# tatsuya-ogawa/GaussianSplattingMlx

Measured on AMD Instinct MI355X. Metric: train views/sec (full step: fwd + L1/DSSIM loss + bwd + Adam + densify/prune at the reference cadence), Lego 800x800 300k Gaussians, higher is better.
Workload: dtype f32

## Files before the change

gaussiansplattingmlx_amd/csrc/blend_v2.hip:

```cpp
#include "gs_ctx.h"
#include "gs_bwd_prep.h"
#include "gs_cull.h"
#include "gs_wavesum.h"

namespace gs {

constexpr int BLK = 16;
constexpr uint32_t CKPT_POOL_MAX = 8;
static inline uint32_t ckpt_pool(uint32_t partSlots, uint32_t waves)
{
    const uint32_t perWave = partSlots / (waves / 8u + 1u);
    return perWave >= CKPT_POOL_MAX ? CKPT_POOL_MAX : (perWave < 1u ? 1u : perWave);
}

struct Rec {
    float mx, my, c00, c01, c10, c11, r, g, b, op, depth;
};

#ifndef GS_FWD_PREFETCH
#define GS_FWD_PREFETCH 1
#endif

typedef float f4 __attribute__((ext_vector_type(4)));
typedef float f2 __attribute__((ext_vector_type(2)));
// ... 587 lines not shown
        const int by = b / blocksX, bx = b - by * blocksX;
        const int tile = ((by * BLK) / tileH) * gridW + (bx * BLK) / tileW;
        const uint32_t start = __builtin_amdgcn_readfirstlane(tileRanges[2 * tile]);
        const uint32_t end = __builtin_amdgcn_readfirstlane(tileRanges[2 * tile + 1]);
        const uint32_t count = end > start ? end - start : 0u;
        const uint32_t sbase = __builtin_amdgcn_readfirstlane(segBase[b]);

        int X0, Y0, XL, YL;
        gs_block_pixels(vg, bx, by, W, H, X0, Y0, XL, YL);
        const int x = X0 + k * 8 + (lane & 7), y = Y0 + h * 8 + (lane >> 3);
        const bool in = x < XL && y < YL;
        const float px = (float)x, py = (float)y;
        const float qx0 = (float)(X0 + k * 8), qx1 = qx0 + 7.0f, qy0 = (float)(Y0 + h * 8), qy1 = qy0 + 7.0f;
        float T = in ? 1.0f : 0.0f;
        float cr = 0.f, cg = 0.f, cb = 0.f, dd = 0.f;
        uint32_t nc = 0;

        const uint32_t* __restrict__ idx = sortedIdx + start;
        auto save_state_vals = [&](uint32_t i, float sT, float sr, float sgr, float sb, float sd) {
            if (poolNext == poolEnd) {
                poolNext = qslotCap;
                for (uint32_t t = 0; t < 8u && poolNext == qslotCap; t++) {
                    const uint32_t yy = (part + t) & 7u;
                    if ((partsEmpty >> yy) & 1u) continue;
                    uint32_t base = 0;
                    if (lane == 0) base = atomicAdd(&counters[GS_CNT_QSLOTS + yy], ckptPool);
                    base = __builtin_amdgcn_readfirstlane(base);
                    if (base + ckptPool <= qslotPart) poolNext = gridDim.x * 4u * qslotOwn + yy * qslotPart + base;
                    else {
                        partsEmpty |= 1u << yy;
                        if (lane == 0) atomicSub(&counters[GS_CNT_QSLOTS + yy], ckptPool);
                    }
                }
                if (poolNext == qslotCap && partsEmpty == 0xFFu && lane == 0) atomicAdd(&counters[GS_CNT_QSLOTS + part], ckptPool);
                poolEnd = poolNext + ckptPool;
            }
            const uint32_t phys = poolNext++;
            const uint32_t vslot = sbase + i / SEG - 1;
            if (phys < qslotCap && vslot < segCap) {
                if (lane == 0) segSlot[(size_t)vslot * 4 + (h * 2 + k)] = phys;
                float* st = segState + (size_t)phys * (statePlanes * 64) + lane;
                if (sT >= 1e-4f) {
                    st[0] = sT; st[64] = sr; st[128] = sgr; st[192] = sb;
                    if (DEPTH && statePlanes == 5) st[256] = sd;
                }
            } else if (lane == 0) {
                counters[GS_CNT_OVERFLOW] = 1u;
                hostWords[4] = 2u;
            }
        };
        auto save_state = [&](uint32_t i) { save_state_vals(i, T, cr, cg, cb, dd); };
        struct Pre {
            float aclamp, r, g, b, depth;
            uint32_t ncv;
        };
        auto stage_compact = [&](f4* sl, const RecV& v, uint32_t c0) -> uint32_t {
            const float qmin = rect_min_q(v.a.z, v.a.w, v.b.x, v.b.y, qx0 - v.a.x, qx1 - v.a.x, qy0 - v.a.y, qy1 - v.a.y);
            const bool keep = (c0 + lane < count) && !(qmin > CULL_QMIN);
            const unsigned long long m = __ballot(keep);
            const uint32_t ps = (uint32_t)__popcll(m & ((1ull << lane) - 1ull));
            if (keep) {
                sl[ps * 3] = v.a; sl[ps * 3 + 1] = v.b;
                sl[ps * 3 + 2] = (f4){v.c.x, v.c.y, v.c.z, __uint_as_float(c0 + (uint32_t)lane + 1u)};
            }
            const uint32_t n = (uint32_t)__popcll(m), n4 = (n + 3u) & ~3u;
            if ((uint32_t)lane < n4 - n) {
                const f4 z = (f4){0.f, 0.f, 0.f, 0.f};
                sl[(n + lane) * 3] = z; sl[(n + lane) * 3 + 1] = z;
                sl[(n + lane) * 3 + 2] = (f4){0.f, 0.f, 0.f, __uint_as_float(min(c0 + 64u, count))};
            }
            return n4;
        };
        auto pre = [&](const f4* sl, uint32_t j, Pre& o) {
            const Rec s = unpack(sl[j * 3], sl[j * 3 + 1], sl[j * 3 + 2]);
            const float dx = px - s.mx, dy = py - s.my;
            const float dxdy = dx * dy, dx2 = dx * dx, dy2 = dy * dy;
            const float q = ((dx2 * s.c00 + dy2 * s.c11) + dxdy * s.c01) + dxdy * s.c10;
            o.aclamp = fminf(gauss_alpha_raw(q, s.op), 0.99f);
            o.r = s.r; o.g = s.g; o.b = s.b; o.depth = s.depth;
            o.ncv = __float_as_uint(sl[j * 3 + 2].w);
        };
        auto post = [&](const Pre& o) {
            const bool a = T >= 1e-4f;
            nc = a ? o.ncv : nc;
            const float alpha = a ? o.aclamp : 0.0f;
            const float wgt = T * alpha;
            cr = fmaf(wgt, o.r, cr); cg = fmaf(wgt, o.g, cg); cb = fmaf(wgt, o.b, cb); if (DEPTH) dd = fmaf(wgt, o.depth, dd);
            T = T * (1.0f - alpha);
        };
        auto any_live = [&]() { return __any(T >= 1e-4f); };
        auto trips_abs = [&](const f4* sl, uint32_t n, uint32_t c0, float* park) {
            park[lane] = cr; park[64 + lane] = cg; park[128 + lane] = cb; if (DEPTH) park[192 + lane] = dd;
            cr = 0.f; cg = 0.f; cb = 0.f; dd = 0.f;
            bool live = true;
            for (uint32_t j = 0; j < n && live; j += 4) {
                Pre p0, p1, p2, p3;
                pre(sl, j, p0); pre(sl, j + 1, p1); pre(sl, j + 2, p2); pre(sl, j + 3, p3);
                post(p0); post(p1); post(p2); post(p3);
                live = any_live();
            }
            if (live && T >= 1e-4f) nc = min(c0 + 64u, count);
            cr = park[lane] + cr; cg = park[64 + lane] + cg; cb = park[128 + lane] + cb; if (DEPTH) dd = park[192 + lane] + dd;
        };

        auto chunk_of = [&](uint32_t r) { return 256u * r + 64u * (((uint32_t)hw + r) & 3u); };
        RecV nx = load_chunk(rec12, idx, idxMask, chunk_of(0), count, lane);
        uint32_t gN = load_chunk_index(idx, idxMask, chunk_of(1), count, lane);
        for (uint32_t r = 0; 256u * r < count; r++) {
            if (!any_live()) break;
            const uint32_t s0 = 256u * r;
            const int w = (int)(((uint32_t)hw + r) & 3u);
            const uint32_t c0 = s0 + 64u * (uint32_t)w;
            const uint32_t nParts = min(4u, (count - s0 + 63u) / 64u);
            const bool mine = (uint32_t)w < nParts;
            f4* sl = sg;
            uint32_t n = 0;
            if (mine) n = stage_compact(sl, nx, c0);
            nx = gather_chunk(rec12, gN);
            gN = load_chunk_index(idx, idxMask, chunk_of(r + 2), count, lane);
            if (w == 0) {
                if (statePlanes != 0 && c0 != 0) save_state(c0);
                trips_abs(sl, n, c0, &xPre[hw][0][0]);
            } else if (mine) {
                T = in ? 1.0f : 0.0f; cr = 0.f; cg = 0.f; cb = 0.f; dd = 0.f;
                for (uint32_t j = 0; j < n; j += 4) {
                    Pre p0, p1, p2, p3;
                    pre(sl, j, p0); pre(sl, j + 1, p1); pre(sl, j + 2, p2); pre(sl, j + 3, p3);
#pragma unroll
                    for (int u = 0; u < 4; u++) {
                        const Pre& o = u == 0 ? p0 : u == 1 ? p1 : u == 2 ? p2 : p3;
                        const float wgt = T * o.aclamp;
                        cr = fmaf(wgt, o.r, cr); cg = fmaf(wgt, o.g, cg); cb = fmaf(wgt, o.b, cb); if (DEPTH) dd = fmaf(wgt, o.depth, dd);
                        T = T * (1.0f - o.aclamp);
                    }
                }
            }
            if (mine) { xEnd[w][0][lane] = T; xEnd[w][1][lane] = cr; xEnd[w][2][lane] = cg; xEnd[w][3][lane] = cb; xEnd[w][4][lane] = dd; }
            if (w == 0) xDead[0][5][lane] = __uint_as_float(nc);
            __syncthreads();
            float PT = xEnd[0][0][lane], Pr = xEnd[0][1][lane], Pg = xEnd[0][2][lane], Pb = xEnd[0][3][lane], Pd = xEnd[0][4][lane];
            uint32_t Pnc = __float_as_uint(xDead[0][5][lane]);
            float myPT = 0.0f;
            uint32_t qDone = 1;
            for (;;) {
                int crossedIn = 0;
#pragma unroll
                for (int q = 1; q < 4; q++) {
                    if ((uint32_t)q >= qDone && (uint32_t)q < nParts && !crossedIn) {
                        if (q == w) { myPT = PT; xPre[hw][0][lane] = Pr; xPre[hw][1][lane] = Pg; xPre[hw][2][lane] = Pb; if (DEPTH) xPre[hw][3][lane] = Pd; }
                        if (PT >= 1e-4f) {
                            const float Tend = PT * xEnd[q][0][lane];
                            if (Tend * foldScale >= 1e-4f) {
                                Pr = fmaf(PT, xEnd[q][1][lane], Pr); Pg = fmaf(PT, xEnd[q][2][lane], Pg); Pb = fmaf(PT, xEnd[q][3][lane], Pb);
                                if (DEPTH) Pd = fmaf(PT, xEnd[q][4][lane], Pd);
                                PT = Tend;
                                Pnc = min(s0 + 64u * (uint32_t)(q + 1), count);
                            } else crossedIn = q;
                        }
                        if (!crossedIn) qDone = (uint32_t)q + 1u;
                    }
                }
                if (!__syncthreads_or(crossedIn != 0)) break;
                if (w != 0 && mine && __any(crossedIn == w)) {
                    T = crossedIn == w ? PT : 0.0f; cr = Pr; cg = Pg; cb = Pb; dd = Pd; nc = 0;
                    trips_abs(sl, n, c0, &xDead[w][1][0]);
                    if (crossedIn == w) {
                        xDead[w][0][lane] = T; xDead[w][1][lane] = cr; xDead[w][2][lane] = cg; xDead[w][3][lane] = cb; xDead[w][4][lane] = dd;
                        xDead[w][5][lane] = __uint_as_float(nc);
                    }
                }
                __syncthreads();
                bool again = false;
                if (crossedIn) {
                    PT = xDead[crossedIn][0][lane]; Pr = xDead[crossedIn][1][lane]; Pg = xDead[crossedIn][2][lane];
                    Pb = xDead[crossedIn][3][lane]; Pd = xDead[crossedIn][4][lane]; Pnc = __float_as_uint(xDead[crossedIn][5][lane]);
                    qDone = (uint32_t)crossedIn + 1u;
                    again = PT >= 1e-4f && qDone < nParts;
                    if (!again) qDone = 4u;
                }
                if (!__syncthreads_or(again)) break;
            }
            if (statePlanes != 0 && w != 0 && mine && __any(myPT >= 1e-4f))
                save_state_vals(c0, myPT, xPre[hw][0][lane], xPre[hw][1][lane], xPre[hw][2][lane], DEPTH ? xPre[hw][3][lane] : 0.0f);
            T = PT; cr = Pr; cg = Pg; cb = Pb; dd = Pd; nc = Pnc;
        }
        if (hw == 0) {
            if (cutStore && any_live() && lane == 0 && cutStore[tile] != 0u) hostWords[0] = 1u;
            const int xe = X0 + k * 8 + (lane & 7), ye = Y0 + h * 8 + (lane >> 3);
            if (xe < XL && ye < YL) {
                const size_t pix = (size_t)ye * W + xe;
                float bg0, bg1, bg2;
                gs_bg_terms(bgc, T, bg0, bg1, bg2);
                outColor[3 * pix] = cr + bg0; outColor[3 * pix + 1] = cg + bg1; outColor[3 * pix + 2] = cb + bg2;
                if (DEPTH) outDepth[pix] = dd;
                outAlpha[pix] = 1.0f - T; lastContrib[pix] = nc; finalT[pix] = T;
            }
            uint32_t m = (xe < XL && ye < YL) ? nc : 0u;
#pragma unroll
            for (int d = 32; d >= 1; d >>= 1) m = max(m, (uint32_t)__shfl_xor((int)m, d, 64));
            if (lane == 0 && m) atomicMax(&blockWork[b], m);
        }
    }
}


struct RecB {
    float mx, my, A, B, Dq, r, g, b, op, depth;
};
__device__ __forceinline__ RecB unpack_b(const f4 a, const f4 b, const f4 c)
{
    RecB r;
    r.mx = a.x; r.my = a.y; r.A = a.z; r.B = a.w;
    r.Dq = b.x; r.r = b.z; r.g = b.w;
    r.b = c.x; r.op = c.y; r.depth = c.z;
    return r;
}
constexpr float EXP_INV_C1 = -1.3862943611198906f;

struct PairB {
    f2 dx, dxdy, dx2, e2;
    float dy, dy2;
};
__device__ __forceinline__ void pair_exponent_bwd(const RecB& s, f2 px, float py, PairB& o)
{
    o.dx = px - splat2(s.mx);
    o.dy = py - s.my;
    o.dxdy = o.dx * splat2(o.dy);
    o.dx2 = o.dx * o.dx;
    o.dy2 = o.dy * o.dy;
    o.e2 = fma2(o.dxdy, splat2(s.B), fma2(o.dx2, splat2(s.A), splat2(o.dy2 * s.Dq)));
}

struct PairState {
    f2 px, Ts, Q;
    f2 cCx, cCy, cCz, cD;
    float py;
    uint32_t nc0, nc1;
};

template <bool DEPTH, bool ABSGRAD, int NACC>
__device__ __forceinline__ void pair_bwd(const RecB& s, uint32_t i, const PairB& e, PairState& p, f2 (&acc)[NACC])
{
    static_assert(NACC == (ABSGRAD ? 12 : 10), "ten sums, twelve with the absolute ones");
    const f2 G = (f2){__builtin_amdgcn_exp2f(e.e2.x), __builtin_amdgcn_exp2f(e.e2.y)};
    const f2 raw = splat2(s.op) * G;
    const bool a0 = i < p.nc0, a1 = i < p.nc1;
    f2 alpha;
    alpha.x = a0 ? fminf(raw.x, 0.99f) : 0.0f;
    alpha.y = a1 ? fminf(raw.y, 0.99f) : 0.0f;
    const f2 contrib = p.Ts * alpha;
    const f2 S = fma2(p.cCx, splat2(s.r), fma2(p.cCy, splat2(s.g),
                      DEPTH ? fma2(p.cCz, splat2(s.b), p.cD * splat2(s.depth)) : p.cCz * splat2(s.b)));
    p.Q = fma2(-contrib, S, p.Q);
    const f2 oma = splat2(1.0f) - alpha;
    const f2 owed = p.Q * (f2){__builtin_amdgcn_rcpf(oma.x), __builtin_amdgcn_rcpf(oma.y)};
    const f2 dAlpha = fma2(p.Ts, S, -owed);
    f2 gate;
    gate.x = (a0 && !(raw.x > 0.99f)) ? dAlpha.x : 0.0f;
    gate.y = (a1 && !(raw.y > 0.99f)) ? dAlpha.y : 0.0f;
    const f2 hh = gate * raw;
    acc[0] = fma2(hh, e.dx, acc[0]);
    acc[1] = fma2(hh, splat2(e.dy), acc[1]);
    acc[2] = fma2(e.dx2, hh, acc[2]);
    acc[3] = fma2(e.dxdy, hh, acc[3]);
    acc[4] = fma2(splat2(e.dy2), hh, acc[4]);
    acc[5] = fma2(G, gate, acc[5]);
    acc[6] = fma2(contrib, p.cCx, acc[6]);
    acc[7] = fma2(contrib, p.cCy, acc[7]);
    acc[8] = fma2(contrib, p.cCz, acc[8]);
    if (DEPTH) acc[9] = fma2(contrib, p.cD, acc[9]);
    if constexpr (ABSGRAD) {
        const float hB = 0.5f * s.B;
        const float tx = hB * e.dy, ty = s.Dq * e.dy;
        const float u0 = fmaf(e.dx.x, s.A, tx), u1 = fmaf(e.dx.y, s.A, tx);
        const float v0 = fmaf(e.dx.x, hB, ty), v1 = fmaf(e.dx.y, hB, ty);
        acc[10].x = fmaf(fabsf(hh.x), fabsf(u0), acc[10].x);
        acc[10].y = fmaf(fabsf(hh.y), fabsf(u1), acc[10].y);
        acc[11].x = fmaf(fabsf(hh.x), fabsf(v0), acc[11].x);
        acc[11].y = fmaf(fabsf(hh.y), fabsf(v1), acc[11].y);
    }
    p.Ts = p.Ts * oma;
}

template <int SEG, bool DEPTH, bool ABSGRAD>
__global__ __launch_bounds__(64) void blend_bwd_v2_kernel(
    int W, int H, int tileW, int tileH, int gridW, int blocksX, GsBackground bgc, const float4* __restrict__ rec12,
    const uint32_t* __restrict__ sortedIdx, uint32_t idxMask, const uint32_t* __restrict__ tileRanges,
    const uint32_t* __restrict__ itemRow, const uint4* __restrict__ segSlot, uint32_t qslotCap, int statePlanes,
    const uint32_t* __restrict__ blockWork,
    const uint32_t* __restrict__ itemBlock, uint32_t* __restrict__ counters, uint32_t* __restrict__ bwdQueue, uint32_t nq,
    const float* __restrict__ cotColor,
    const float* __restrict__ cotDepth, const float* __restrict__ cotAlpha, const float* __restrict__ outColor,
    const float* __restrict__ outDepth, const float* __restrict__ outAlpha, const uint32_t* __restrict__ lastContrib,
    const float* __restrict__ finalT, const float* __restrict__ segState, float* __restrict__ gradAcc16, GsVirtGeom vg)
{
    __shared__ float part[SEG][16];
    __shared__ f4 sg[192];
    const int lane = threadIdx.x;
    const uint32_t nItems = __builtin_amdgcn_readfirstlane(counters[GS_CNT_ITEMS]);
    const uint32_t xcd = blockIdx.x % nq, slot = blockIdx.x / nq;
    const uint32_t perQ = (nItems + nq - 1u) / nq;
    const uint32_t staticPerQ = min(gridDim.x / nq, perQ);
    uint32_t dead = 0;
    for (bool first = true;; first = false) {
        uint32_t item = 0xFFFFFFFFu;
        if (first && slot < staticPerQ) item = xcd * perQ + slot;
        else {
            for (uint32_t t = 0; t < nq && item == 0xFFFFFFFFu; t++) {
                const uint32_t y = (xcd + t) % nq;
                if ((dead >> y) & 1u) continue;
                uint32_t k = 0;
                if (lane == 0) k = atomicAdd(&bwdQueue[y * 32u], 1u);
                k = __builtin_amdgcn_readfirstlane(k);
                const uint32_t idx = staticPerQ + k;
                if (idx < perQ && y * perQ + idx < nItems) item = y * perQ + idx;
                else dead |= 1u << y;
            }
        }
        if (item == 0xFFFFFFFFu || item >= nItems) {
            if (first) continue;
            break;
        }
        const uint32_t packed = __builtin_amdgcn_readfirstlane(itemBlock[item]);
        const uint32_t row = __builtin_amdgcn_readfirstlane(itemRow[item]);
        const int b = (int)(packed >> 10);
        const uint32_t seg = packed & 1023u;
        const int by = b / blocksX, bx = b - by * blocksX;
        const int tile = ((by * BLK) / tileH) * gridW + (bx * BLK) / tileW;
        const uint32_t start = __builtin_amdgcn_readfirstlane(tileRanges[2 * tile]);
        const uint32_t work = __builtin_amdgcn_readfirstlane(blockWork[b]);
        const uint32_t i0 = seg * SEG, i1 = min(i0 + SEG, work);
        uint32_t qslot[4] = {0, 0, 0, 0};
        if (seg != 0) {
            const uint4 q4 = segSlot[row];
            qslot[0] = __builtin_amdgcn_readfirstlane(q4.x); qslot[1] = __builtin_amdgcn_readfirstlane(q4.y);
            qslot[2] = __builtin_amdgcn_readfirstlane(q4.z); qslot[3] = __builtin_amdgcn_readfirstlane(q4.w);
        }

        int BX0, BY0, BXL, BYL;
        gs_block_pixels(vg, bx, by, W, H, BX0, BY0, BXL, BYL);
        PairState ps[2];
#pragma unroll
        for (int h = 0; h < 2; h++) {
            PairState& p = ps[h];
            const int y = BY0 + h * 8 + (lane >> 3);
            p.py = (float)y;
            p.Ts = p.Q = p.cCx = p.cCy = p.cCz = p.cD = splat2(0.f);
            uint32_t ncs[2] = {0, 0};
#pragma unroll
            for (int k = 0; k < 2; k++) {
                const int x = BX0 + k * 8 + (lane & 7);
                p.px[k] = (float)x;
                if (x < BXL && y < BYL) {
                    const size_t pix = (size_t)y * W + x;
                    const uint32_t n = lastContrib[pix];
                    if (n > i0) {
                        ncs[k] = n;
                        const float gx = cotColor[3 * pix], gy = cotColor[3 * pix + 1], gz = cotColor[3 * pix + 2];
                        const float gd = DEPTH ? cotDepth[pix] : 0.0f;
                        p.cCx[k] = gx; p.cCy[k] = gy; p.cCz[k] = gz; p.cD[k] = gd;
                        const float cA = cotAlpha ? cotAlpha[pix] : 0.0f;
                        const float Tn = finalT[pix];
                        float bg0, bg1, bg2;
                        gs_bg_terms(bgc, Tn, bg0, bg1, bg2);
                        const float cTn = -cA + gs_bg_cot(bgc, gx, gy, gz);
                        const float sc = (1.0f - outAlpha[pix]) / Tn;
                        float T0 = 1.0f, s0 = 0.0f, s1 = 0.0f, s2 = 0.0f, s3 = 0.0f;
                        const uint32_t phys = qslot[h * 2 + k];
                        if (seg != 0 && phys < qslotCap) {
                            const float* st = segState + (size_t)phys * (statePlanes * 64) + lane;
                            T0 = st[0]; s0 = st[64]; s1 = st[128]; s2 = st[192];
                            if (DEPTH) s3 = st[256];
                        }
                        const float d0 = (outColor[3 * pix] - bg0) - s0, d1 = (outColor[3 * pix + 1] - bg1) - s1, d2 = (outColor[3 * pix + 2] - bg2) - s2;
                        const float owedC = fmaf(gx, d0, fmaf(gy, d1, fmaf(gz, d2, DEPTH ? gd * (outDepth[pix] - s3) : 0.0f)));
                        p.Ts[k] = sc * T0;
                        p.Q[k] = sc * (owedC + Tn * cTn);
                    }
                }
            }
            p.nc0 = ncs[0]; p.nc1 = ncs[1];
        }

        uint32_t hm0 = max(ps[0].nc0, ps[0].nc1), hm1 = max(ps[1].nc0, ps[1].nc1);
#pragma unroll
        for (int d = 32; d >= 1; d >>= 1) {
            hm0 = max(hm0, (uint32_t)__shfl_xor((int)hm0, d, 64));
            hm1 = max(hm1, (uint32_t)__shfl_xor((int)hm1, d, 64));
        }
        const uint32_t* __restrict__ idx = sortedIdx + start;
        const uint32_t n = i1 - i0;
        for (uint32_t r = lane; r < n * 4; r += 64) reinterpret_cast<f4*>(&part[0][0])[r] = (f4){0.f, 0.f, 0.f, 0.f};
        const float bx0 = (float)BX0, bx1 = bx0 + 15.0f, by0 = (float)BY0;
        for (uint32_t c0 = i0; c0 < i1; c0 += 64) {
            uint32_t nEff;
            {
                const RecV v = load_chunk(rec12, idx, idxMask, c0, i1, lane);
                const float X0 = bx0 - v.a.x, X1 = bx1 - v.a.x, Yt = by0 - v.a.y;
                const uint32_t li = c0 + (uint32_t)lane;
                const bool far0 = li >= hm0 || rect_min_q(v.a.z, v.a.w, v.b.x, v.b.y, X0, X1, Yt, Yt + 7.0f) > CULL_QMIN;
                const bool far1 = li >= hm1 || rect_min_q(v.a.z, v.a.w, v.b.x, v.b.y, X0, X1, Yt + 8.0f, Yt + 15.0f) > CULL_QMIN;
                const bool keep = (c0 + lane < i1) && !(far0 && far1);
                const unsigned long long m = __ballot(keep);
                const uint32_t pos = (uint32_t)__popcll(m & ((1ull << lane) - 1ull));
                if (keep) {
                    const uint32_t tag = (c0 - i0 + (uint32_t)lane) | (far0 ? 256u : 0u) | (far1 ? 512u : 0u);
                    sg[pos * 3] = (f4){v.a.x, v.a.y, v.a.z * EXP_C1, (v.a.w + v.b.x) * EXP_C1};
                    sg[pos * 3 + 1] = (f4){v.b.y * EXP_C1, 0.0f, v.b.z, v.b.w};
                    sg[pos * 3 + 2] = (f4){v.c.x, v.c.y, v.c.z, __uint_as_float(tag)};
                }
                nEff = (uint32_t)__popcll(m);
            }
          for (uint32_t jl = 0; jl < nEff; jl++) {
            const f4 rc = sg[jl * 3 + 2];
            const uint32_t tag = __builtin_amdgcn_readfirstlane(__float_as_uint(rc.w));
            const uint32_t i = i0 + (tag & 255u);
            const RecB s = unpack_b(sg[jl * 3], sg[jl * 3 + 1], rc);
            PairB e0, e1;
            const bool k0 = (tag & 256u) != 0, k1 = (tag & 512u) != 0;
            if (!k0) pair_exponent_bwd(s, ps[0].px, ps[0].py, e0);
            if (!k1) pair_exponent_bwd(s, ps[1].px, ps[1].py, e1);
            constexpr int NACC = ABSGRAD ? 12 : 10;
            f2 acc2[NACC];
#pragma unroll
            for (int q = 0; q < NACC; q++) acc2[q] = splat2(0.0f);
            if (!k0) pair_bwd<DEPTH, ABSGRAD, NACC>(s, i, e0, ps[0], acc2);
            if (!k1) pair_bwd<DEPTH, ABSGRAD, NACC>(s, i, e1, ps[1], acc2);
            float acc[NACC];
#pragma unroll
            for (int q = 0; q < NACC; q++) acc[q] = acc2[q].x + acc2[q].y;
            float w;
            if constexpr (ABSGRAD) w = wave_sum12_transposed<!DEPTH>(acc);
            else w = wave_sum10_transposed<!DEPTH>(acc);
            if (lane == 20) w = s.A * EXP_INV_C1;
            if (lane == 28) w = s.Dq * EXP_INV_C1;
            if (lane == 52) w = s.B * EXP_INV_C1;
            if ((lane & 3) == 0) part[i - i0][lane >> 2] = w;
          }
        }
        __builtin_amdgcn_s_waitcnt(0xc07f);
        __builtin_amdgcn_wave_barrier();
        constexpr uint32_t NCOL = ABSGRAD ? 13u : 11u;
        for (uint32_t e = lane; e < n * NCOL; e += 64) {
            const uint32_t j = e / NCOL, q = e - j * NCOL;
            float v;
            if (ABSGRAD && q >= 11) {
                v = part[j][q == 11 ? 12 : 14] * -EXP_INV_C1;
            } else if (q < 2) {
                const float a1 = -0.5f * part[j][0], a2 = -0.5f * part[j][2], cs = part[j][13];
                v = q == 0 ? -(2.0f * part[j][5] * a1 + cs * a2) : -(2.0f * part[j][7] * a2 + cs * a1);
            } else {
                const uint32_t src = (0x6a4b98331ull >> ((q - 2) * 4)) & 15u;
                v = (DEPTH || q != 10) ? part[j][src] : 0.0f;
                if (q < 6) v *= -0.5f;
            }
            if (v != 0.0f) atomicAdd(&gradAcc16[(size_t)(idx[i0 + j] & idxMask) * 16 + (ABSGRAD && q >= 11 ? q + 1 : q)], v);
        }
        __builtin_amdgcn_s_waitcnt(0xc07f);
        __builtin_amdgcn_wave_barrier();
    }
}

constexpr int SEGLEN = GS_SEG_LEN;
bool blend_forward_v2_wide(const gs_ctx* c)
{
    if (c->fwdTrace || !c->fwdQuadrants) return false;
    return c->fwdWide == 1 || (c->fwdWide < 0 && c->numPixBlocks * 4 <= c->numCUs * 4 * c->fwdWavesPerSimd);
}
bool blend_forward_v2_pair_decide(const gs_ctx* c)
{
    if (c->fwdTrace || !c->fwdQuadrants || blend_forward_v2_wide(c)) return false;
    if (c->fwdPair >= 0) return c->fwdPair != 0;
    const unsigned long long lastM = c->missHost ? c->missHost[8] : 0u;
    return c->numPixBlocks > 0 && lastM / (unsigned long long)c->numPixBlocks >= 4500ull;
}
bool blend_forward_v2_pair(const gs_ctx* c)
{
    return c->fwdPairNow;
}
int blend_forward_v2_grid(const gs_ctx* c)
{
    const int fwdItems = c->numPixBlocks * 4;
    const int fwdGrid = blend_forward_v2_wide(c) ? c->numCUs * GS_V2W_WGS
                        : blend_forward_v2_pair(c) ? c->numCUs * (c->fwdPair > 1 ? c->fwdPair : GS_V2P_WGS)
                                                   : c->numCUs * 4 * c->fwdWavesPerSimd;
    return fwdGrid > fwdItems ? fwdItems : fwdGrid;
}

void fill_seg_base(gs_ctx* c, SegBaseArgs& a)
{
    a.nBlocks = c->numPixBlocks; a.blocksX = c->blocksX; a.tileW = c->tileW; a.tileH = c->tileH; a.gridW = c->gridW;
    a.tileRanges = c->tileRanges; a.tileTotal = nullptr;
    a.segBase = c->segBase; a.blockWork = c->blockWork; a.counters = c->counters; a.workHint = c->workHint;
    a.blockOrder = c->blockOrder; a.queueStart = (uint32_t)blend_forward_v2_grid(c); a.fwdQueue = c->fwdQueue; a.nq = c->fwdQueues; a.spatial = c->fwdSpatial;
}

int launch_blend_forward_v2(gs_ctx* c, float* outColor, float* outDepth, float* outAlpha)
{
    const int planes = c->depthGradient && outDepth ? 5 : 4;
    c->fwd.statePlanes = planes;
    const int blocksX = c->blocksX, nBlocks = c->numPixBlocks;
    const int nItems = nBlocks * 4, grid = blend_forward_v2_grid(c);
    if (c->segBaseDone) c->segBaseDone = false;
    else {
        SegBaseArgs sa;
        fill_seg_base(c, sa);
        hipLaunchKernelGGL(seg_base_kernel<SEGLEN>, dim3(1), dim3(1024), 0, c->stream, sa);
    }
    const uint32_t* cuts = c->fwd.cutsActive ? c->fwd.cutStore : nullptr;
    const uint32_t qcap = (uint32_t)(c->qslotCap * 5 / c->fwd.statePlanes);
    c->fwd.qslotCap = qcap;
    uint32_t own = (uint32_t)(((unsigned long long)qcap * 3ull / 4ull) / (unsigned long long)grid);
    if (own > 32u) own = 32u;
    c->fwd.qslotStatic = own * (uint32_t)grid;
    const uint32_t partSlots = (qcap - c->fwd.qslotStatic) / 8u;
    if (c->poisonCheckpoints && c->segState)
        GS_HIP_CHECK(c, hipMemsetAsync(c->segState, 0xFF, (size_t)c->qslotCap * 5 * 64 * sizeof(float), c->stream));
    if (blend_forward_v2_wide(c)) {
        uint32_t ownW = (uint32_t)(((unsigned long long)qcap * 3ull / 4ull) / (unsigned long long)(grid * 4));
        if (ownW > 32u) ownW = 32u;
        c->fwd.qslotStatic = ownW * (uint32_t)grid * 4u;
        const uint32_t partW = (qcap - c->fwd.qslotStatic) / 8u;
        auto kw = outDepth ? blend_fwd_v2w_kernel<SEGLEN, true> : blend_fwd_v2w_kernel<SEGLEN, false>;
        hipLaunchKernelGGL(kw, dim3(grid), dim3(256), 0, c->stream, c->W, c->H, c->tileW,
                           c->tileH, c->gridW, blocksX, nItems, c->bg, reinterpret_cast<const float4*>(c->packed12),
                           c->sortedRaw, c->idxMask, c->tileRanges, c->segBase, (uint32_t)c->segCap, c->renderOnly ? 0 : c->fwd.statePlanes, outColor, outDepth,
                           outAlpha, c->lastContrib, c->finalT, c->segState, c->segSlot, qcap, ownW, partW, ckpt_pool(partW, (uint32_t)grid * 4u), c->blockWork, c->counters, c->fwdQueue,
                           (uint32_t)c->fwdQueues, c->blockOrder, cuts, c->missDev, c->fwdFoldScale, c->virt);
        GS_HIP_CHECK(c, hipGetLastError());
        if (c->renderOnly) c->fwd.statePlanes = 0;
        return GS_OK;
    }
    if (blend_forward_v2_pair(c)) {
        auto kp = outDepth ? blend_fwd_v2p_kernel<SEGLEN, true> : blend_fwd_v2p_kernel<SEGLEN, false>;
        hipLaunchKernelGGL(kp, dim3(grid), dim3(128), 0, c->stream, c->W, c->H, c->tileW,
                           c->tileH, c->gridW, blocksX, nItems, c->bg, reinterpret_cast<const float4*>(c->packed12),
                           c->sortedRaw, c->idxMask, c->tileRanges, c->segBase, (uint32_t)c->segCap, c->renderOnly ? 0 : c->fwd.statePlanes, outColor, outDepth,
                           outAlpha, c->lastContrib, c->finalT, c->segState, c->segSlot, qcap, own, partSlots, ckpt_pool(partSlots, (uint32_t)grid), c->blockWork, c->counters, c->fwdQueue, (uint32_t)c->fwdQueues, c->blockOrder,
                           cuts, c->missDev, c->virt);
        GS_HIP_CHECK(c, hipGetLastError());
        if (c->renderOnly) c->fwd.statePlanes = 0;
        return GS_OK;
    }
    auto kern = outDepth ? blend_fwd_v2q_kernel<SEGLEN, true> : blend_fwd_v2q_kernel<SEGLEN, false>;
    hipLaunchKernelGGL(kern, dim3(grid / 4), dim3(256), 0, c->stream, c->W, c->H, c->tileW,
                       c->tileH, c->gridW, blocksX, nItems, c->bg, reinterpret_cast<const float4*>(c->packed12),
                       c->sortedRaw, c->idxMask, c->tileRanges, c->segBase, (uint32_t)c->segCap, c->renderOnly ? 0 : c->fwd.statePlanes, outColor, outDepth,
                       outAlpha, c->lastContrib, c->finalT, c->segState, c->segSlot, qcap, own, partSlots, ckpt_pool(partSlots, (uint32_t)grid), c->blockWork, c->counters, c->fwdQueue, (uint32_t)c->fwdQueues, c->blockOrder,
                       c->fwdTrace, cuts, c->missDev, (uint32_t)c->fwdSlowSlot, c->virt);
    GS_HIP_CHECK(c, hipGetLastError());
    if (c->renderOnly) c->fwd.statePlanes = 0;
    return GS_OK;
}

void fill_bwd_prep(gs_ctx* c, int N, uint32_t queueStart, BwdPrepArgs& p)
{
    p.nBlocks = c->numPixBlocks;
    p.blockWork = c->fwd.blockWork;
    p.itemBlock = c->itemBlock;
    p.itemRow = c->itemRow;
    p.segBase = c->segBase;
    p.itemCap = (uint32_t)c->itemCap;
    p.counters = c->counters;
    p.queueStart = queueStart;
    p.bwdQueue = c->bwdQueue;
    p.clearBuf = reinterpret_cast<float4*>(c->gradAcc16);
    p.clearCount = (size_t)N * 4;
    p.cutStore = c->fwd.cutStore;
    p.cutsInForce = c->fwd.cutsActive ? 1 : 0;
    p.tileRanges = c->tileRanges;
    p.sortedIdx = c->sortedRaw;
    p.idxMask = c->idxMask;
    p.rec12 = c->packed12;
}

int blend_backward_v2_grid(const gs_ctx* c)
{
    int grid = c->numCUs * c->bwdWavesPerCu;
    if ((long long)grid > c->itemCap) grid = (int)c->itemCap;
    return grid < 1 ? 1 : grid;
}

int launch_blend_backward_v2(gs_ctx* c, int N, const float* cotColor, const float* cotDepth, const float* cotAlpha,
                             const float* outColor, const float* outDepth, const float* outAlpha, bool absgrad)
{
    const int blocksX = c->blocksX, nBlocks = c->numPixBlocks;
    const int grid = blend_backward_v2_grid(c);
    BwdPrepArgs prep;
    fill_bwd_prep(c, N, (uint32_t)grid, prep);
    const bool prepared = c->fwd.bwdPrepared && c->fwd.preparedQueueStart == (uint32_t)grid && c->fwd.preparedN == N;
    c->fwd.bwdPrepared = false;
    if (!prepared) {
        const int cutBlocks = prep.cutStore ? gs_div_up(nBlocks, 1024) : 0;
        const int clearBlocks = (int)((prep.clearCount + 8191) / 8192 < 1024 ? (prep.clearCount + 8191) / 8192 : 1024);
        hipLaunchKernelGGL(bwd_items_kernel<SEGLEN>, dim3(GS_ITEM_PARTS + cutBlocks + clearBlocks), dim3(1024), 0, c->stream, prep, cutBlocks);
    }
    auto kern = absgrad ? (cotDepth ? blend_bwd_v2_kernel<SEGLEN, true, true> : blend_bwd_v2_kernel<SEGLEN, false, true>)
                        : (cotDepth ? blend_bwd_v2_kernel<SEGLEN, true, false> : blend_bwd_v2_kernel<SEGLEN, false, false>);
    hipLaunchKernelGGL(kern, dim3(grid), dim3(64), 0, c->stream, c->W, c->H, c->tileW, c->tileH,
                       c->gridW, blocksX, c->fwd.bg, reinterpret_cast<const float4*>(c->packed12), c->sortedRaw,
                       c->idxMask, c->tileRanges, c->itemRow, reinterpret_cast<const uint4*>(c->segSlot), c->fwd.qslotCap, c->fwd.statePlanes, c->fwd.blockWork, c->itemBlock, c->counters, c->bwdQueue, (uint32_t)c->bwdQueues, cotColor,
                       cotDepth, cotAlpha, outColor, outDepth, outAlpha, c->lastContrib, c->finalT, c->segState,
                       c->gradAcc16, c->virt);
    GS_HIP_CHECK(c, hipGetLastError());
    return GS_OK;
}

}
```

Before: 644.2.

## Flush backward gradients per chunk over kept Gaussians only, caching global index

The backward blend kernel now writes gradient atomics after each 64-Gaussian chunk and only for the kept (non-culled) Gaussians, instead of zeroing the whole part buffer and flushing every Gaussian in the tile range at the end. The global Gaussian index is stored in the shared record, so the flush no longer re-reads sortedIdx. Per-lane column mapping is precomputed once outside the loop, and the flush is skipped for columns that are zero when depth is disabled. This cuts LDS zeroing, useless atomics for culled Gaussians and index reloads, at the cost of extra wave barriers per chunk.

```diff
diff --git a/gaussiansplattingmlx_amd/csrc/blend_v2.hip b/gaussiansplattingmlx_amd/csrc/blend_v2.hip
--- a/gaussiansplattingmlx_amd/csrc/blend_v2.hip
+++ b/gaussiansplattingmlx_amd/csrc/blend_v2.hip
@@ -913,6 +913,14 @@
     const uint32_t perQ = (nItems + nq - 1u) / nq;
     const uint32_t staticPerQ = min(gridDim.x / nq, perQ);
     uint32_t dead = 0;
+    constexpr uint32_t NC = (ABSGRAD ? 13u : 11u) - (DEPTH ? 0u : 1u), RPI = 64u / NC;
+    const uint32_t fRow = (uint32_t)lane / NC, fc = (uint32_t)lane - fRow * NC;
+    const uint32_t fq = (!DEPTH && fc >= 10u) ? fc + 1u : fc;
+    const bool fMean = fq < 2u, fAbs = ABSGRAD && fq >= 11u;
+    const uint32_t fSrc = fMean ? (fq == 0u ? 5u : 7u) : fAbs ? (fq == 11u ? 12u : 14u) : (uint32_t)((0x6a4b98331ull >> ((fq - 2u) * 4u % 64u)) & 15u);
+    const uint32_t fCol = fAbs ? fq + 1u : fq;
+    const float fMul = fAbs ? -EXP_INV_C1 : -0.5f;
+    const bool fScaled = fAbs || (fq >= 2u && fq < 6u);
     for (bool first = true;; first = false) {
         uint32_t item = 0xFFFFFFFFu;
         if (first && slot < staticPerQ) item = xcd * perQ + slot;
@@ -1000,13 +1008,12 @@
             hm1 = max(hm1, (uint32_t)__shfl_xor((int)hm1, d, 64));
         }
         const uint32_t* __restrict__ idx = sortedIdx + start;
-        const uint32_t n = i1 - i0;
-        for (uint32_t r = lane; r < n * 4; r += 64) reinterpret_cast<f4*>(&part[0][0])[r] = (f4){0.f, 0.f, 0.f, 0.f};
         const float bx0 = (float)BX0, bx1 = bx0 + 15.0f, by0 = (float)BY0;
         for (uint32_t c0 = i0; c0 < i1; c0 += 64) {
             uint32_t nEff;
             {
-                const RecV v = load_chunk(rec12, idx, idxMask, c0, i1, lane);
+                const uint32_t gi = load_chunk_index(idx, idxMask, c0, i1, lane);
+                const RecV v = gather_chunk(rec12, gi);
                 const float X0 = bx0 - v.a.x, X1 = bx1 - v.a.x, Yt = by0 - v.a.y;
                 const uint32_t li = c0 + (uint32_t)lane;
                 const bool far0 = li >= hm0 || rect_min_q(v.a.z, v.a.w, v.b.x, v.b.y, X0, X1, Yt, Yt + 7.0f) > CULL_QMIN;
@@ -1017,7 +1024,7 @@
                 if (keep) {
                     const uint32_t tag = (c0 - i0 + (uint32_t)lane) | (far0 ? 256u : 0u) | (far1 ? 512u : 0u);
                     sg[pos * 3] = (f4){v.a.x, v.a.y, v.a.z * EXP_C1, (v.a.w + v.b.x) * EXP_C1};
-                    sg[pos * 3 + 1] = (f4){v.b.y * EXP_C1, 0.0f, v.b.z, v.b.w};
+                    sg[pos * 3 + 1] = (f4){v.b.y * EXP_C1, __uint_as_float(gi), v.b.z, v.b.w};
                     sg[pos * 3 + 2] = (f4){v.c.x, v.c.y, v.c.z, __uint_as_float(tag)};
                 }
                 nEff = (uint32_t)__popcll(m);
@@ -1048,27 +1055,25 @@
             if (lane == 52) w = s.B * EXP_INV_C1;
             if ((lane & 3) == 0) part[i - i0][lane >> 2] = w;
           }
-        }
-        __builtin_amdgcn_s_waitcnt(0xc07f);
-        __builtin_amdgcn_wave_barrier();
-        constexpr uint32_t NCOL = ABSGRAD ? 13u : 11u;
-        for (uint32_t e = lane; e < n * NCOL; e += 64) {
-            const uint32_t j = e / NCOL, q = e - j * NCOL;
-            float v;
-            if (ABSGRAD && q >= 11) {
-                v = part[j][q == 11 ? 12 : 14] * -EXP_INV_C1;
-            } else if (q < 2) {
-                const float a1 = -0.5f * part[j][0], a2 = -0.5f * part[j][2], cs = part[j][13];
-                v = q == 0 ? -(2.0f * part[j][5] * a1 + cs * a2) : -(2.0f * part[j][7] * a2 + cs * a1);
-            } else {
-                const uint32_t src = (0x6a4b98331ull >> ((q - 2) * 4)) & 15u;
-                v = (DEPTH || q != 10) ? part[j][src] : 0.0f;
-                if (q < 6) v *= -0.5f;
-            }
-            if (v != 0.0f) atomicAdd(&gradAcc16[(size_t)(idx[i0 + j] & idxMask) * 16 + (ABSGRAD && q >= 11 ? q + 1 : q)], v);
-        }
-        __builtin_amdgcn_s_waitcnt(0xc07f);
-        __builtin_amdgcn_wave_barrier();
+          __builtin_amdgcn_s_waitcnt(0xc07f);
+          __builtin_amdgcn_wave_barrier();
+          for (uint32_t jb = 0; jb < nEff; jb += RPI) {
+            const uint32_t jl = jb + fRow;
+            if (fRow < RPI && jl < nEff) {
+                const float* const rec = reinterpret_cast<const float*>(&sg[jl * 3]);
+                const uint32_t g = __float_as_uint(rec[5]), j = __float_as_uint(rec[11]) & 255u;
+                const float* const pr = part[j];
+                const float s0 = pr[0], s2 = pr[2], cs = pr[13], src = pr[fSrc];
+                const float own = -0.5f * (fq == 0u ? s0 : s2), oth = -0.5f * (fq == 0u ? s2 : s0);
+                const float vm = -(2.0f * src * own + cs * oth);
+                const float vs = fScaled ? src * fMul : src;
+                const float v = fMean ? vm : vs;
+                if (v != 0.0f) atomicAdd(&gradAcc16[(size_t)g * 16 + fCol], v);
+            }
+          }
+          __builtin_amdgcn_s_waitcnt(0xc07f);
+          __builtin_amdgcn_wave_barrier();
+        }
     }
 }
 
```

Result: faster. 651.2 (median of 6 runs) (+1.1%).
